# AmnonDrory/PointDSC

Hardware: AMD Instinct MI355X
Metric: correspondence-pairs/sec through NSM (N=1k/5k) at 1/2/4/8 GPUs; 3DMatch recall parity (higher is better)
Workload: dtype f32 (3xf16-split contractions); 1 GPU; synthetic random correspondences N=1000 (3dmatch-like, 30% inliers), 128 scan pairs per GPU per step, full PointDSC testing forward (12 layers x 128 ch, trained synthetic weights, classifier rescaled by synthetic.BENCH_CLS for tie-free seed ranking); num_corr=1000, global_batch=128, parallelism=dp1 (independent pairs)

## Files before the change

pointdsc_amd/csrc/attention.hip:

```cpp
#include "abi.hpp"
#include "encoder_row.hpp"

namespace pdsc {

static __global__ __launch_bounds__(256) void vexp_kernel(const float *__restrict__ v, int N, int ld, int Npad,
                                                         float *__restrict__ vexp) {
    __shared__ float part[4];
    const int t = blockIdx.x, b = blockIdx.y, tid = threadIdx.x;
    float m = 0.0f;
    for (int e = tid; e < H3_TILE * CH; e += 256) {
        const int row = t * H3_TILE + e / CH;
        if (row < N) m = fmaxf(m, fabsf(v[((size_t)b * ld + row) * CH + e % CH]));
    }
    m = wave_max(m);
    if ((tid & 63) == 0) part[tid >> 6] = m;
    __syncthreads();
    if (tid == 0) vexp[(size_t)b * (Npad / H3_TILE) + t] = (float)h3_vexp(fmaxf(fmaxf(part[0], part[1]), fmaxf(part[2], part[3])));
}

static __global__ void split_qkv_kernel(const float *__restrict__ q, const float *__restrict__ k,
                                 const float *__restrict__ v, const float *__restrict__ vexp, int B, int N,
                                 int ld, int Npad, _Float16 *__restrict__ Qs, _Float16 *__restrict__ Ks,
                                 _Float16 *__restrict__ Vs) {
    const size_t i = (size_t)blockIdx.x * blockDim.x + threadIdx.x;
// ... 13 lines not shown
    const float ev = vexp[(size_t)b * (Npad / H3_TILE) + row / H3_TILE];
    split_h(in ? ldexpf(v[src], (int)ev) : 0.0f, hi, lo);
    Vs[pb + vs_off(row, 0, c)] = hi;
    Vs[pb + vs_off(row, 1, c)] = lo;
}

hipError_t launch_attention(const EncoderPlan &plan, const void *q, const void *k, const void *v, const float *vexp,
                            const float *M, float *opart, float *ml, hipStream_t s, Ragged rg, int layer) {
    const dim3 grid(plan.workgroups());
    const _Float16 *qs = static_cast<const _Float16 *>(q), *ks = static_cast<const _Float16 *>(k),
                   *vs = static_cast<const _Float16 *>(v);
    const AttnGridH3 g = plan_grid_h3(plan, rg, layer);
    const bool packed = plan.m_layout == M_PACKED;
    switch (plan.kind) {
    case ATT_W64_SK:
        hipLaunchKernelGGL((attention_w64_sk_kernel<true>), grid, dim3(W64_NW * 64), W64_LDS, s, qs, ks, vs, vexp, M, g,
                           plan.sk_wgs, opart, ml);
        break;
    case ATT_W64:
        hipLaunchKernelGGL((attention_w64_kernel<true>), grid, dim3(W64_NW * 64), W64_LDS, s, qs, ks, vs, vexp, M, g,
                           opart, ml);
        break;
    case ATT_F32: {
        const AttnGrid gf{plan.B, plan.N, plan.Npad, plan.nqb, plan.nsplit, plan.sps, rg.nv};
        hipLaunchKernelGGL((attention_kernel_t<ATT_NW, ATT_F32_KTS, false, true>), grid, dim3(ATT_NW * 64),
                           (attention_lds_bytes<ATT_NW, ATT_F32_KTS>()), s, static_cast<const float *>(q),
                           static_cast<const float *>(k), static_cast<const float *>(v), M, gf, opart, ml);
        break;
    }
    case ATT_H3_WS:
        if (plan.vfold) return hipErrorInvalidValue;
        with_int<2, 4>(plan.ws, [&](auto ws) {
            with_bool(packed, [&](auto pk) {
                constexpr int WS = decltype(ws)::value;
                hipLaunchKernelGGL((attention_h3_ws_kernel<WS, decltype(pk)::value>), grid, dim3(WS * 64),
                                   attention_h3_ws_lds_bytes<WS>(), s, qs, ks, vs, vexp, M, g, opart, ml);
// ... 111 lines not shown
```

pointdsc_amd/csrc/attention_w64.hpp:

```cpp
#pragma once
#include "attention_h3.hpp"

namespace pdsc {

template <typename F, int... I> PDSC_DEV void static_for_(F &f, std::integer_sequence<int, I...>) {
    (f(std::integral_constant<int, I>{}), ...);
}
template <int N, typename F> PDSC_DEV void static_for(F &&f) { static_for_(f, std::make_integer_sequence<int, N>{}); }

template <typename T> PDSC_DEV void w64_pin(T &x) { asm volatile("" : "+v"(x)); }

constexpr int W64_NW = 4;
constexpr int W64_QW = 64;
constexpr int W64_QPB = W64_NW * W64_QW;
constexpr int W64_NSLOT = 4;
constexpr size_t W64_RING = (size_t)W64_NSLOT * (H3_KTB + H3_VTB);
constexpr int W64_MAXT = 1024;
constexpr size_t W64_LDS = W64_RING + W64_MAXT * sizeof(float);

constexpr int W64_AO = 0, W64_AQ = 128;
#define W64_AGPRS "a0","a1","a2","a3","a4","a5","a6","a7","a8","a9","a10","a11","a12","a13","a14","a15","a16","a17","a18","a19","a20","a21","a22","a23","a24","a25","a26","a27","a28","a29","a30","a31","a32","a33","a34","a35","a36","a37","a38","a39","a40","a41","a42","a43","a44","a45","a46","a47","a48","a49","a50","a51","a52","a53","a54","a55","a56","a57","a58","a59","a60","a61","a62","a63","a64","a65","a66","a67","a68","a69","a70","a71","a72","a73","a74","a75","a76","a77","a78","a79","a80","a81","a82","a83","a84","a85","a86","a87","a88","a89","a90","a91","a92","a93","a94","a95","a96","a97","a98","a99","a100","a101","a102","a103","a104","a105","a106","a107","a108","a109","a110","a111","a112","a113","a114","a115","a116","a117","a118","a119","a120","a121","a122","a123","a124","a125","a126","a127","a128","a129","a130","a131","a132","a133","a134","a135","a136","a137","a138","a139","a140","a141","a142","a143","a144","a145","a146","a147","a148","a149","a150","a151","a152","a153","a154","a155","a156","a157","a158","a159","a160","a161","a162","a163","a164","a165","a166","a167","a168","a169","a170","a171","a172","a173","a174","a175","a176","a177","a178","a179","a180","a181","a182","a183","a184","a185","a186","a187","a188","a189","a190","a191","a192","a193","a194","a195","a196","a197","a198","a199","a200","a201","a202","a203","a204","a205","a206","a207","a208","a209","a210","a211","a212","a213","a214","a215","a216","a217","a218","a219","a220","a221","a222","a223","a224","a225","a226","a227","a228","a229","a230","a231","a232","a233","a234","a235","a236","a237","a238","a239","a240","a241","a242","a243","a244","a245","a246","a247","a248","a249","a250","a251","a252","a253","a254","a255"
PDSC_DEV void w64_claim_agprs() { asm volatile("" ::: W64_AGPRS); }

template <int QA> PDSC_DEV void w64_kq0(f32x16 &c, const f16x8 &k) {
    asm volatile("v_mfma_f32_32x32x16_f16 %0, %1, a[%c2:%c3], 0" : "=&v"(c) : "v"(k), "i"(QA), "i"(QA + 3));
}
template <int QA> PDSC_DEV void w64_kq(f32x16 &c, const f16x8 &k) {
    asm volatile("v_mfma_f32_32x32x16_f16 %0, %1, a[%c2:%c3], %0" : "+v"(c) : "v"(k), "i"(QA), "i"(QA + 3));
}
template <int QA> PDSC_DEV void w64_kq_last(f32x16 &c, const f16x8 &k) {
    asm volatile("v_mfma_f32_32x32x16_f16 %0, %1, a[%c2:%c3], %0\n\ts_nop 11" : "+v"(c) : "v"(k), "i"(QA), "i"(QA + 3));
}
template <int U, int J> PDSC_DEV void w64_qk_step(f32x16 &S, const f16x8 (&kf)[2]) {
// ... 39 lines not shown
template <int R, int G> PDSC_DEV void w64_mload_row(__amdgpu_buffer_rsrc_t r, uint32_t voff) {
    asm volatile("buffer_load_dwordx4 v[%c0:%c1], %2, %3, 0 offen offset:%c4" ::"i"(R + 4 * G), "i"(R + 4 * G + 3),
                 "v"(voff), "s"(r), "i"(32 * G)
                 : "memory");
}
template <int R, int G> PDSC_DEV void w64_mload_col(__amdgpu_buffer_rsrc_t r, uint32_t voff) {
    asm volatile("buffer_load_dword v%c0, %4, %5, 0 offen offset:%c6\n\t"
                 "buffer_load_dword v%c1, %4, %5, 0 offen offset:%c7\n\t"
                 "buffer_load_dword v%c2, %4, %5, 0 offen offset:%c8\n\t"
                 "buffer_load_dword v%c3, %4, %5, 0 offen offset:%c9" ::"i"(R + 4 * G), "i"(R + 4 * G + 1),
                 "i"(R + 4 * G + 2), "i"(R + 4 * G + 3), "v"(voff), "s"(r), "i"(1024 * G), "i"(1024 * G + 128),
                 "i"(1024 * G + 256), "i"(1024 * G + 384)
                 : "memory");
}
template <int N> PDSC_DEV void w64_vmwait() { asm volatile("s_waitcnt vmcnt(%0)" ::"n"(N) : "memory"); }
PDSC_DEV void w64_mwait_after(bool other_keyrows) {
    if (other_keyrows)
        w64_vmwait<8 + 16>();
    else
        w64_vmwait<8 + 4>();
}
template <int R> PDSC_DEV float w64_fma_m(float sv, float mb) {
    float p;
    asm volatile("v_fma_f32 %0, v%c1, %2, -%3" : "=v"(p) : "i"(R), "v"(sv), "v"(mb));
    return p;
}
template <int R> PDSC_DEV void w64_mul_m(float &p) { asm volatile("v_mul_f32 %0, v%c1, %0" : "+v"(p) : "i"(R)); }

#ifdef W64_STAMPS
constexpr int W64_ST_PER_TILE = 6, W64_ST_TILES = 40, W64_ST_WGS = 64;
constexpr int W64_ST_PER_WAVE = W64_ST_PER_TILE * W64_ST_TILES + 8;
constexpr size_t W64_ST_LDS = (size_t)W64_NW * W64_ST_PER_WAVE * 8;
static __device__ unsigned long long g_w64_stamps[W64_ST_WGS * W64_NW * W64_ST_PER_WAVE];
#define W64_ST(i)                                                                                   \
    do {                                                                                            \
        __builtin_amdgcn_sched_barrier(0);                                                          \
// ... 9 lines not shown
    } while (0)
#endif

PDSC_DEV void w64_cvt_hi(float x0, float x1, uint32_t &hi) {
    asm volatile("v_cvt_pk_f16_f32 %0, %1, %2" : "=v"(hi) : "v"(x0), "v"(x1));
}
PDSC_DEV void w64_mix_lo(float x0, uint32_t hi, uint32_t &lo) {
    asm volatile("v_fma_mixlo_f16 %0, %1, 1.0, -%2 op_sel_hi:[0,0,1]" : "=&v"(lo) : "v"(x0), "v"(hi));
}
PDSC_DEV void w64_mix_hi(float x1, uint32_t hi, uint32_t &lo) {
    asm volatile("v_fma_mixhi_f16 %0, %1, 1.0, -%2 op_sel:[0,0,1] op_sel_hi:[0,0,1]" : "+v"(lo) : "v"(x1), "v"(hi));
}

inline AttnGridH3 attention_w64_grid(int B, int N, int slots) { return attention_h3_grid<W64_QPB / 32>(B, N, slots); }

PDSC_DEV void attention_w64_core(const _Float16 *__restrict__ Qs, const _Float16 *__restrict__ Ks,
                                 const _Float16 *__restrict__ Vs, const float *__restrict__ vexp,
                                 const float *__restrict__ M, const AttnGridH3 &g, const AttnBlock &blk, char *smem,
                                 int wave, int lane, float (&m_run)[2], float (&l_run)[2]) {
    const int b = blk.b, qb = blk.qb, split = blk.split;
    const int N = g.n(b), Npad = g.Npad;
    const int h = lane >> 5;
    const int q0 = qb * W64_QPB + wave * W64_QW;
    const int nst = (N + H3_TILE - 1) / H3_TILE;
    const int st0 = blk.st1 >= 0 ? blk.st0 : split * g.sps, st1 = blk.st1 >= 0 ? blk.st1 : min(nst, st0 + g.sps);

    const char *Kp = reinterpret_cast<const char *>(Ks + (size_t)b * Npad * 2 * CH);
    const char *Vp = reinterpret_cast<const char *>(Vs + (size_t)b * Npad * 2 * CH);
    const int mnt = mpack_ntile(g.N);
    const size_t mper = mpack_floats(g.N);
#ifdef W64_EXP_MSHARED
    const __amdgpu_buffer_rsrc_t rM = h3_rsrc(M, (uint32_t)(mper * 4u));
#else
    const __amdgpu_buffer_rsrc_t rM = h3_rsrc(M + (size_t)b * mper, (uint32_t)(mper * 4u));
#endif
    const float *vexp_b = vexp + (size_t)b * (Npad / H3_TILE);
    const __amdgpu_buffer_rsrc_t rK = h3_rsrc(Kp, (uint32_t)Npad * H3_ROWB), rV = h3_rsrc(Vp, (uint32_t)Npad * H3_ROWB);

#ifdef W64_STAMPS
    unsigned long long *st_lds = reinterpret_cast<unsigned long long *>(smem + W64_LDS) + wave * W64_ST_PER_WAVE;
    const unsigned long long st_c0 = __builtin_amdgcn_s_memtime(), st_r0 = __builtin_amdgcn_s_memrealtime();
#endif
    w64_claim_agprs();
    w64_claim_vm();
    static_for<128>([&](auto ic) { w64_zero_a<W64_AO + decltype(ic)::value>(); });
#pragma unroll
    for (int u = 0; u < 2; ++u) {
        m_run[u] = -INFINITY;
        l_run[u] = 0.0f;
    }
    if (st0 >= st1) return;
    static_for<2>([&](auto uc) {
        constexpr int u = decltype(uc)::value;
        const _Float16 *qt =
            Qs + (size_t)b * Npad * 2 * CH + (size_t)(min(q0 + 32 * u, Npad - 32) >> 5) * H3_TILE_H;
        static_for<8>([&](auto jc) {
            constexpr int j = decltype(jc)::value;
            w64_load_q<W64_AQ + 64 * u + 8 * j>(qt + h3_frag(j, 0, lane));
            w64_load_q<W64_AQ + 64 * u + 8 * j + 4>(qt + h3_frag(j, 1, lane));
        });
    });

    auto slot_of = [&](int st) { return smem + ((st - st0) & (W64_NSLOT - 1)) * (H3_KTB + H3_VTB); };
    constexpr int DMA_PW = (H3_KTB + H3_VTB) / 1024 / W64_NW;
    static_assert(H3_KTB == H3_VTB && W64_NW * DMA_PW == 2 * H3_KTB / 1024, "K / V split over the waves");
    const __amdgpu_buffer_rsrc_t rS = wave < W64_NW / 2 ? rK : rV;
    const int pbase = (wave * DMA_PW) % (H3_KTB / 1024);
    auto stage_piece = [&](int st, int i) {
        char *dst = slot_of(st) + (wave * DMA_PW + i) * 1024;
        __builtin_amdgcn_raw_ptr_buffer_load_lds(rS, (__attribute__((address_space(3))) void *)dst, 16, 16 * lane,
                                                 st * H3_KTB + (pbase + i) * 1024, 0, 0);
    };
    const int qt0 = q0 >> 5;
    const uint32_t vcol = (uint32_t)(4 * h * MPACK_T + (lane & 31)) * 4u;
    const uint32_t vrow = (uint32_t)((lane & 31) * MPACK_T + 4 * h) * 4u;
    auto keyrows = [&](int st, int u) { return st <= qt0 + u; };
    auto kr = [&](auto shc, int st, int u) {
        constexpr int SH = decltype(shc)::value;
        if constexpr (SH == 1)
            return true;
        else if constexpr (SH == 2)
            return false;
        else
            return keyrows(st, u);
    };
    using SH0 = std::integral_constant<int, 0>;
    using SH1 = std::integral_constant<int, 1>;
    using SH2 = std::integral_constant<int, 2>;
    auto load_mq = [&](auto shc, auto msc, auto uc, auto gc, int st) {
        constexpr int R = W64_VM + 32 * decltype(msc)::value + 16 * decltype(uc)::value, gg = decltype(gc)::value;
        const int qt = qt0 + decltype(uc)::value;
        if (kr(shc, st, decltype(uc)::value))
            w64_mload_col<R, gg>(rM, vcol + (uint32_t)mpack_tile(st, qt, mnt) * (MPACK_T * MPACK_T * 4u));
        else
            w64_mload_row<R, gg>(rM, vrow + (uint32_t)mpack_tile(qt, st, mnt) * (MPACK_T * MPACK_T * 4u));
    };
    const float *ev_lds = reinterpret_cast<const float *>(smem + W64_RING);
    auto load_ev = [&](int st) { return ev_lds[st]; };

#ifdef W64_EXP_NO_LDSREAD
    bool lds_once = true;
#endif
    auto kread = [&](const char *Kl, int j, f16x8(&f)[2]) {
#ifdef W64_EXP_NO_LDSREAD
        if (!lds_once) return;
#endif
        f[0] = *reinterpret_cast<const f16x8 *>(Kl + 2 * h3_frag(j, 0, lane));
        f[1] = *reinterpret_cast<const f16x8 *>(Kl + 2 * h3_frag(j, 1, lane));
    };
    auto vread = [&](const char *Vl, int i, f16x8(&f)[2]) {
#ifdef W64_EXP_NO_LDSREAD
        if (!lds_once) return;
// ... 36 lines not shown
        } else if constexpr (k == 21) {
            a.mx = halves_max(a.mx);
            w64_pin(a.mx);
        } else if constexpr (k == 22) {
            a.resc = __any(a.mx > H3_DEFER + (float)H3_PSHIFT - ev);
        }
    };
    auto rebase = [&](auto uc, SmA &a) {
        constexpr int u = decltype(uc)::value;
        if (a.resc) {
            const float m_new = fmaxf(m_run[u], a.mx + a.mb0);
            const float alpha = __builtin_amdgcn_exp2f(m_run[u] - m_new);
            const float dm = m_new - m_run[u];
            m_run[u] = m_new;
            l_run[u] *= alpha;
            static_for<64>([&](auto ic) { w64_scale_a<W64_AO + 64 * u + decltype(ic)::value>(alpha); });
            asm volatile("s_nop 1");
#pragma unroll
            for (int r = 0; r < 16; ++r) a.p[r] -= dm;
        }
    };
    auto sm1_first = [&](int u, const f32x16 &S, auto mrc, float ev, int key0, SmA &a) {
        constexpr int MR = decltype(mrc)::value;
        const float scale = ATT_QFMA ? 1.0f : H3_QSCALE;
        float mx = -INFINITY;
#pragma unroll
        for (int r = 0; r < 16; ++r) a.p[r] = S[r] * scale;
        static_for<16>([&](auto rc) { w64_mul_m<MR + decltype(rc)::value>(a.p[decltype(rc)::value]); });
        if (key0 + 32 > N) {
#pragma unroll
            for (int r = 0; r < 16; ++r)
// ... 86 lines not shown
                    w64_kq<QH>(S, f[1]);
            } else if constexpr (m == 1) {
                w64_kq<QL>(S, f[0]);
            } else {
                if constexpr (j == 7)
                    w64_kq_last<QH>(S, f[0]);
                else
                    w64_kq<QH>(S, f[0]);
            }
            slice(kc);
            __builtin_amdgcn_sched_barrier(0);
        });
    };
    auto pv_region = [&](auto uc, const char *Vl, const f16x8 (&ph)[2], const f16x8 (&pl)[2], auto nextread, auto slice) {
        constexpr int U = decltype(uc)::value;
        static_for<24>([&](auto kc) {
            constexpr int k = decltype(kc)::value, i = k / 3, m = k % 3;
            if constexpr (m == 0) {
                if constexpr (i + 2 < 8)
                    vread(Vl, i + 2, vf.f[(i + 2) % 3]);
                else
                    nextread(std::integral_constant<int, i - 6>{});
            }
            constexpr int OA = W64_AO + 64 * U + 16 * (i >> 1);
            const f16x8(&f)[2] = vf.f[i % 3];
            if constexpr (m == 0)
                w64_vp<OA>(f[0], pl[i & 1]);
            else if constexpr (m == 1)
                w64_vp<OA>(f[1], ph[i & 1]);
            else
                w64_vp<OA>(f[0], ph[i & 1]);
            slice(kc);
            __builtin_amdgcn_sched_barrier(0);
        });
    };
    auto next_k = [&](const char *Kl) { return [&, Kl](auto ic) { kread(Kl, decltype(ic)::value, kf.f[decltype(ic)::value]); }; };
    auto next_v = [&](const char *Vl) { return [&, Vl](auto ic) { vread(Vl, decltype(ic)::value, vf.f[decltype(ic)::value]); }; };
    auto none = [](auto) {};

    auto mid_barrier = [&](auto shc, int tn) {
        if (kr(shc, tn, 0))
            __builtin_amdgcn_s_waitcnt(0x4F74);
        else
            __builtin_amdgcn_s_waitcnt(0x0F78);
        __builtin_amdgcn_s_barrier();
    };

    using MSX = std::integral_constant<int, 0>;
    using MSY = std::integral_constant<int, 1>;
    auto mregs = [](auto msc, auto uc) { return std::integral_constant<int, W64_VM + 32 * decltype(msc)::value + 16 * decltype(uc)::value>{}; };
    float eX, eY;
    f32x16 S[2];
    SmA sa[2];
    SmB sb;
    f16x8 ph[2][2], pl[2][2];

    auto issue_half = [&](auto shc, auto kc, auto hc, int tn, int td, auto msn) {
        constexpr int k = decltype(kc)::value, half = decltype(hc)::value;
#ifndef W64_EXP_NO_M
        if constexpr (k % 3 == 1 && k <= 10) load_mq(shc, msn, hc, std::integral_constant<int, k / 3>{}, tn);
#endif
#ifndef W64_EXP_NO_DMA
        if constexpr (k % 3 == 1 && k >= 13) stage_piece(td, 4 * half + (k - 13) / 3);
#endif
    };
    using H0 = std::integral_constant<int, 0>;
    using H1 = std::integral_constant<int, 1>;

#pragma unroll
    for (int i = 0; i < DMA_PW; ++i) stage_piece(st0, i);
#pragma unroll
    for (int i = 0; i < DMA_PW; ++i) stage_piece(st0 + 1, i);
    static_for<2>([&](auto uc) { static_for<4>([&](auto gc) { load_mq(SH0{}, MSX{}, uc, gc, st0); }); });
    {
        float *evw = reinterpret_cast<float *>(smem + W64_RING);
        for (int i = threadIdx.x; i < Npad / H3_TILE; i += W64_NW * 64) evw[i] = vexp_b[i];
    }
    w64_vmwait<0>();
    __builtin_amdgcn_s_waitcnt(0x0070);
    __builtin_amdgcn_s_barrier();
    eX = load_ev(st0);

    {
        const int t = st0, key0 = t * H3_TILE;
        const char *L = slot_of(t);
        kread(L, 0, kf.f[0]);
        kread(L, 1, kf.f[1]);
        qk_region(std::integral_constant<int, 0>{}, L, S[0], none, none);
        static_for<24>([&](auto kc) { issue_half(SH0{}, kc, H0{}, min(t + 1, st1 - 1), t + 2, MSY{}); });
        eY = load_ev(min(t + 1, st1 - 1));
// ... 5 lines not shown
        mid_barrier(SH0{}, min(t + 1, st1 - 1));
        pv_region(std::integral_constant<int, 0>{}, L + H3_KTB, ph[0], pl[0], next_k(slot_of(t + 1)),
                  [&](auto kc) { issue_half(SH0{}, kc, H1{}, min(t + 1, st1 - 1), t + 2, MSY{}); });
        sm1_first(1, S[1], mregs(MSX{}, H1{}), eX, key0, sa[1]);
    }
    auto tile = [&](int t, auto msc, float &ec, float &ep, auto msn, float &en, auto shc) {
        const int key0 = t * H3_TILE;
        const int si = W64_ST_PER_TILE * min(t - st0, 39);
        (void)si;
        W64_ST(si);
        const char *L = slot_of(t), *Lp = slot_of(t - 1);
        qk_region(std::integral_constant<int, 0>{}, L, S[0], next_v(Lp + H3_KTB),
                  [&](auto kc) { sm2_slice(kc, 1, sa[1], ep, sb, ph[1], pl[1]); });
        W64_ST(si + 1);
        pv_region(std::integral_constant<int, 1>{}, Lp + H3_KTB, ph[1], pl[1], next_k(L), [&](auto kc) {
            if constexpr (decltype(kc)::value == 0) w64_mwait_after(kr(shc, t, 1));
            if constexpr (decltype(kc)::value == 2) en = load_ev(min(t + 1, st1 - 1));
            sm1_slice(kc, 0, S[0], mregs(msc, H0{}), ec, key0, sa[0]);
            issue_half(shc, kc, H0{}, min(t + 1, st1 - 1), t + 2, msn);
        });
        rebase(std::integral_constant<int, 0>{}, sa[0]);
        W64_ST(si + 2);
        qk_region(std::integral_constant<int, 1>{}, L, S[1], next_v(L + H3_KTB),
                  [&](auto kc) { sm2_slice(kc, 0, sa[0], ec, sb, ph[0], pl[0]); });
        W64_ST(si + 3);
        mid_barrier(shc, min(t + 1, st1 - 1));
        W64_ST(si + 4);
        pv_region(std::integral_constant<int, 0>{}, L + H3_KTB, ph[0], pl[0], next_k(slot_of(t + 1)), [&](auto kc) {
            if constexpr (decltype(kc)::value == 0) w64_mwait_after(kr(shc, min(t + 1, st1 - 1), 0));
            sm1_slice(kc, 1, S[1], mregs(msc, H1{}), ec, key0, sa[1]);
            issue_half(shc, kc, H1{}, min(t + 1, st1 - 1), t + 2, msn);
        });
        rebase(std::integral_constant<int, 1>{}, sa[1]);
        W64_ST(si + 5);
    };
#ifdef W64_EXP_NO_LDSREAD
    lds_once = false;
#endif
    int t = st0 + 1;
    for (; t + 1 < st1; t += 2) {
        auto shape = [&](int tt) { return min(tt + 1, st1 - 1) <= qt0 ? 1 : (tt >= qt0 + 2 ? 2 : 0); };
        const int s0 = shape(t), s1 = shape(t + 1);
        auto two = [&](auto shc) {
            tile(t, MSY{}, eY, eX, MSX{}, eX, shc);
// ... 29 lines not shown
        const unsigned long long st_c1 = __builtin_amdgcn_s_memtime(), st_r1 = __builtin_amdgcn_s_memrealtime();
        if (lane == 0) {
            st_lds[W64_ST_PER_WAVE - 4] = st_c0;
            st_lds[W64_ST_PER_WAVE - 3] = st_c1;
            st_lds[W64_ST_PER_WAVE - 2] = st_r0;
            st_lds[W64_ST_PER_WAVE - 1] = st_r1;
        }
        const int wg = blockIdx.x;
        if (wg < W64_ST_WGS)
            for (int i = lane; i < W64_ST_PER_WAVE; i += 64)
                g_w64_stamps[(wg * W64_NW + wave) * W64_ST_PER_WAVE + i] = st_lds[i];
    }
#endif
}

template <int U> PDSC_DEV void w64_read_o(f32x16 (&O)[4]) {
    static_for<64>([&](auto ic) {
        constexpr int i = decltype(ic)::value;
        O[i >> 4][i & 15] = w64_read_a<W64_AO + 64 * U + i>();
    });
}

PDSC_DEV void w64_store_partial(const AttnGridH3 &g, const AttnBlock &blk, float *__restrict__ opart,
                                float *__restrict__ ml, int wave, int lane, const float (&m_run)[2],
                                const float (&l_run)[2]) {
    const int Npad = g.Npad, h = lane >> 5;
    const size_t obase = (size_t)(blk.b * g.nsplit + blk.split) * Npad;
    static_for<2>([&](auto uc) {
        constexpr int u = decltype(uc)::value;
        const int q0 = blk.qb * W64_QPB + wave * W64_QW + 32 * u, qq = q0 + (lane & 31);
        f32x16 O[4];
        w64_read_o<u>(O);
        if (q0 < Npad) {
            float *Ob = opart + obase * CH + (size_t)(q0 >> 5) * (H3_TILE * CH) + 4 * lane;
#pragma unroll
            for (int t = 0; t < 4; ++t)
#pragma unroll
                for (int q = 0; q < 4; ++q)
                    *reinterpret_cast<f32x4 *>(Ob + (4 * t + q) * 256) =
                        f32x4{O[t][4 * q], O[t][4 * q + 1], O[t][4 * q + 2], O[t][4 * q + 3]};
            if (h == 0) {
                ml[(obase + qq) * 2] = (m_run[u] - (float)H3_PSHIFT) * 0.6931471805599453f;
                ml[(obase + qq) * 2 + 1] = l_run[u];
            }
        }
    });
}

template <bool XCD>
__global__ __launch_bounds__(W64_NW * 64, 1) __attribute__((amdgpu_num_vgpr(W64_VM))) void attention_w64_kernel(
    const _Float16 *__restrict__ Qs, const _Float16 *__restrict__ Ks, const _Float16 *__restrict__ Vs,
    const float *__restrict__ vexp, const float *__restrict__ M, AttnGridH3 g, float *__restrict__ opart,
    float *__restrict__ ml) {
    extern __shared__ __attribute__((aligned(16))) char w64smem[];
    const AttnBlock blk = attention_h3_block(g, XCD);
    if (blk.qb * W64_QPB >= g.n(blk.b)) return;
    const int tid = threadIdx.x, wave = __builtin_amdgcn_readfirstlane(tid >> 6), lane = tid & 63;
    float m_run[2], l_run[2];
    attention_w64_core(Qs, Ks, Vs, vexp, M, g, blk, w64smem, wave, lane, m_run, l_run);
    w64_store_partial(g, blk, opart, ml, wave, lane, m_run, l_run);
}

__host__ __device__ inline int w64_sk_owner(long x, long T, int nwg) { return (int)(((x + 1) * nwg - 1) / T); }
inline int w64_sk_nsplit(int B, int nqb, int nst, int nwg) {
    const long T = (long)B * nqb * nst;
    int ns = 1;
    for (long k = 0; k < (long)B * nqb; ++k)
        ns = std::max(ns, w64_sk_owner(k * nst + nst - 1, T, nwg) - w64_sk_owner(k * nst, T, nwg) + 1);
    return ns;
}

PDSC_DEV void w64_zero_partial(const AttnGridH3 &g, int b, int qb, int s, float *__restrict__ opart,
                               float *__restrict__ ml, int tid) {
    const int Npad = g.Npad;
    const size_t obase = (size_t)(b * g.nsplit + s) * Npad;
    const int r0 = qb * W64_QPB, r1 = min(Npad, r0 + W64_QPB);
    f32x4 *Ob = reinterpret_cast<f32x4 *>(opart + (obase + r0) * CH);
    for (int i = tid; i < (r1 - r0) * CH / 4; i += W64_NW * 64) Ob[i] = f32x4{0.0f, 0.0f, 0.0f, 0.0f};
    for (int r = r0 + tid; r < r1; r += W64_NW * 64) {
        ml[(obase + r) * 2] = -INFINITY;
        ml[(obase + r) * 2 + 1] = 0.0f;
    }
}

template <bool XCD>
__global__ __launch_bounds__(W64_NW * 64, 1) __attribute__((amdgpu_num_vgpr(W64_VM))) void attention_w64_sk_kernel(
    const _Float16 *__restrict__ Qs, const _Float16 *__restrict__ Ks, const _Float16 *__restrict__ Vs,
    const float *__restrict__ vexp, const float *__restrict__ M, AttnGridH3 g, int nwg, float *__restrict__ opart,
    float *__restrict__ ml) {
    extern __shared__ __attribute__((aligned(16))) char w64smem[];
    int w = blockIdx.x;
    if (XCD && (nwg & 7) == 0) w = (w & 7) * (nwg >> 3) + (w >> 3);
    const int nst = (g.N + H3_TILE - 1) / H3_TILE;
    const long T = (long)g.B * g.nqb * nst;
    const long hi = (long)(w + 1) * T / nwg;
    const int tid = threadIdx.x, wave = __builtin_amdgcn_readfirstlane(tid >> 6), lane = tid & 63;
    for (long x = (long)w * T / nwg; x < hi;) {
        const int k = (int)(x / nst);
        const long k0 = (long)k * nst, x1 = min(hi, k0 + nst);
        AttnBlock blk{k / g.nqb, k % g.nqb, w - w64_sk_owner(k0, T, nwg)};
        blk.st0 = (int)(x - k0);
        blk.st1 = (int)(x1 - k0);
        __builtin_amdgcn_s_waitcnt(0x0070);
        float m_run[2], l_run[2];
        attention_w64_core(Qs, Ks, Vs, vexp, M, g, blk, w64smem, wave, lane, m_run, l_run);
        w64_store_partial(g, blk, opart, ml, wave, lane, m_run, l_run);
        if (x1 == k0 + nst)
            for (int s = blk.split + 1; s < g.nsplit; ++s) w64_zero_partial(g, blk.b, blk.qb, s, opart, ml, tid);
        x = x1;
    }
}

}
```

pointdsc_amd/csrc/encoder.hip:

```cpp
#include <algorithm>
#include <cstdlib>
#include <mutex>
#include <vector>

#include "abi.hpp"
#include "encoder.hpp"
#include "pw_lds.hpp"

namespace pdsc {

static thread_local int g_diag_qkv_delay = 0;

static bool use_pw2(const Knobs &k, int B, int Npad, bool f32) {
    if (f32 || k.pw2 == 0) return false;
    return k.pw2 == 2 || (long)B * ((Npad + PW2_PTS - 1) / PW2_PTS) >= 320;
}

EncoderPlan plan_encoder(int B, int N, bool f32, bool dense_m_caller, bool allow_fused) {
    const Knobs &k = knobs();
    EncoderPlan p{};
    p.B = B;
    p.N = N;
    p.Npad = round_up(N, QB);
    p.f32 = f32;
// ... 36 lines not shown
        } else {
            p.nw = blocks <= 16 ? k.nw : ATT_NW;
            take(ATT_H3, p.nw == 1   ? attention_h3_grid<1>(B, N, k.target)
                         : p.nw == 2 ? attention_h3_grid<2>(B, N, k.target)
                                     : attention_h3_grid<ATT_NW>(B, N, k.target));
        }
        p.early = p.kind == ATT_H3 && p.sps >= 3;
    }

    p.precombine = k.precombine && !f32 && !fused && p.nsplit >= 16 && blocks <= 16;
    p.m_layout = w64 || !(f32 || dense_m_caller || k.dense_m) ? M_PACKED : M_DENSE;

    p.vfold = k.vfold && allow_fused && !f32 &&
              (fused || (p.pw2 && !p.precombine &&
                         (p.w64() || (p.kind == ATT_H3 && p.nw == ATT_NW))));
    if (fused) {
        p.kind = ATT_FUSED;
        p.nw = PW2_W;
        p.ws = 1;
        p.early = false;
        p.nqb = fg.nqb;
        p.sps = nst;
    }
    if (p.pw2) return p;

    const bool small_tiles = (long)B * (p.Npad / 64) < k.pw_small_limit;
    p.pw_tile = small_tiles ? 32 : 64;
    p.pw_mid8 = !f32 && k.pw_waves8 && (long)B * (p.Npad / 32) <= 256;
    const bool qkv3 = k.pw_qkv_split && 3L * B * (p.Npad / 32) <= 256;
    p.pw_first_qkv3 = !f32 && small_tiles && qkv3;
// ... 519 lines not shown
                split8v(v, xh[2 * t + u], xl[2 * t + u]);
            }
    }
    __syncthreads();
    w2_pcn_qkv<VFOLD>(P, pk, S, cf, d, xh, xl, featL + boff, Q + 2 * boff, K + 2 * boff, V + 2 * boff,
                      vexp + (size_t)b * (Npad / 32), row, active, wave, lane, vpad != 0);
}

template <bool VFOLD>
__global__ __launch_bounds__(PW2_W * 64, PW2_OCC) void pw2_mid_kernel(const float *__restrict__ pk, W2Sched S, PwMsg m,
                                                               PwDense4 d, const float *__restrict__ opart,
                                                               const float *__restrict__ ml, int nsplit, int N,
                                                               int Npad, const float *__restrict__ featL_in,
                                                               float *__restrict__ featL,
                                                               _Float16 *__restrict__ Q, _Float16 *__restrict__ K,
                                                               _Float16 *__restrict__ V, float *__restrict__ vexp) {
    PW2_PROLOGUE
    w2_coef_mid(cf, pk, m, d, tid, VFOLD);
    f16x8 xh[8], xl[8];
    f32x16 a2[2];
    if (active) {
        if constexpr (VFOLD)
            w2_combine_acc(opart, ml, b, nsplit, Npad, row, a2, lane);
        else
            w2_combine(opart, ml, b, nsplit, Npad, row, xh, xl, lane);
    }
    __syncthreads();
    w2_mid_chain<VFOLD>(P, pk, S, cf, m, d, xh, xl, a2, featL_in + boff, featL + boff, Q + 2 * boff, K + 2 * boff,
                        V + 2 * boff, vexp + (size_t)b * (Npad / 32), row, active, wave, lane, true);
}

template <bool PACKED, bool VFOLD>
__global__ __launch_bounds__(PW2_W * 64, PW2_OCC) void attn_pw2_kernel(
    const _Float16 *__restrict__ Qs, const _Float16 *__restrict__ Ks, const _Float16 *__restrict__ Vs,
    const float *__restrict__ vexp_in, const float *__restrict__ M, AttnGridH3 g, const float *__restrict__ pk,
    W2Sched S, PwMsg m, PwDense4 d, float *__restrict__ featL, _Float16 *__restrict__ Q, _Float16 *__restrict__ K,
    _Float16 *__restrict__ V, float *__restrict__ vexp) {
    extern __shared__ __attribute__((aligned(16))) char w2smem[];
    const AttnBlock blk = attention_h3_block(g, true);
    if (blk.qb * PW2_PTS >= g.n(blk.b)) return;
    const int b = blk.b, Npad = g.Npad, tid = threadIdx.x, wave = __builtin_amdgcn_readfirstlane(tid >> 6),
              lane = tid & 63;
    const int row = blk.qb * PW2_PTS + wave * 32 + (lane & 31);
    const bool active = blk.qb * PW2_PTS + wave * 32 < Npad;
// ... 271 lines not shown
        else                                                                                            \
            hipLaunchKernelGGL((K<64, false>), g_, dim3(256), pw_lds<64>(), s, __VA_ARGS__);            \
    } while (0)

static hipError_t launch_pw_first(const EncoderPlan &plan, const float *packed, const PackLayout &lay, const float *corr_pos,
                           float *feat, void *q, void *k, void *v, float *vexp, hipStream_t s, Ragged rg) {
    if (lay.in_dim > IN_LIMIT) return hipErrorInvalidValue;
    const int B = plan.B, N = plan.N, Npad = plan.Npad;
    _Float16 *Q = static_cast<_Float16 *>(q), *K = static_cast<_Float16 *>(k), *V = static_cast<_Float16 *>(v);
    if (plan.pw2) {
        const PwDense4 d = dense4(lay.layer[0], plan.vfold);
        const W2Sched S = sched_qkv(W2Sched{}, d, plan.vfold);
        with_bool(plan.vfold, [&](auto vf) {
            hipLaunchKernelGGL(pw2_first_kernel<decltype(vf)::value>, dim3((Npad + PW2_PTS - 1) / PW2_PTS, B),
                               dim3(PW2_W * 64), PW2_LDS, s, packed, S, lay.l0_w, lay.l0_b, d, corr_pos, lay.in_dim, N,
                               Npad, feat, Q, K, V, vexp, rg.nv, (int)!plan.fused());
        });
        return hipGetLastError();
    }
    if (plan.pw_first_qkv3) {
        hipLaunchKernelGGL((pw_first_kernel<32, false>), dim3(Npad / 32, B, 3), dim3(256), pw_lds<32>(), s, packed,
                           lay.l0_w, lay.l0_b, dense4(lay.layer[0]), corr_pos, lay.in_dim, N, Npad, feat, Q, K, V, vexp,
                           rg.nv);
        return hipGetLastError();
    }
    PW_LAUNCH(pw_first_kernel, Npad, packed, lay.l0_w, lay.l0_b, dense4(lay.layer[0]), corr_pos, lay.in_dim, N, Npad,
              feat, Q, K, V, vexp, rg.nv);
    return hipGetLastError();
}

static hipError_t launch_pw_mid(const EncoderPlan &plan, const float *packed, const PackLayout &lay, int layer,
                         const float *opart, const float *ml, int nsplit, const float *feat_in, float *feat, void *q,
                         void *k, void *v, float *vexp, hipStream_t s) {
    const int delay = g_diag_qkv_delay;
    const int B = plan.B, N = plan.N, Npad = plan.Npad;
    _Float16 *Q = static_cast<_Float16 *>(q), *K = static_cast<_Float16 *>(k), *V = static_cast<_Float16 *>(v);
    if (plan.pw2) {
        const PwMsg m = msg3(lay.layer[layer], plan.vfold);
        const PwDense4 d = dense4(lay.layer[layer + 1], plan.vfold);
        const W2Sched S = sched_qkv(sched_msg(m, plan.vfold), d, plan.vfold);
        with_bool(plan.vfold, [&](auto vf) {
            hipLaunchKernelGGL(pw2_mid_kernel<decltype(vf)::value>, dim3((Npad + PW2_PTS - 1) / PW2_PTS, B),
                               dim3(PW2_W * 64), PW2_LDS, s, packed, S, m, d, opart, ml, nsplit, N, Npad, feat_in, feat, Q,
                               K, V, vexp);
        });
        return hipGetLastError();
    }
    if (plan.pw_mid8) {
        hipLaunchKernelGGL((pw_mid_kernel<32, false, 8>), dim3(Npad / 32, B, plan.pw_mid_qkv3 ? 3 : 1), dim3(512),
                           pw_lds<32>(), s, packed,
                           msg3(lay.layer[layer]), dense4(lay.layer[layer + 1]), opart, ml, nsplit, N, Npad, feat_in,
                           feat, Q, K, V, vexp, delay, (int)plan.pw_prefetch);
        return hipGetLastError();
    }
    PW_LAUNCH(pw_mid_kernel, Npad, packed, msg3(lay.layer[layer]), dense4(lay.layer[layer + 1]), opart, ml, nsplit,
              N, Npad, feat_in, feat, Q, K, V, vexp, 0, 0);
    return hipGetLastError();
}

// ... 281 lines not shown
```

pointdsc_amd/csrc/launch_plan.hpp:

```cpp
#pragma once
#include <algorithm>
#include <cstdlib>

#include "pdsc_internal.hpp"

namespace pdsc {

constexpr int ENC_MAX_PARTS = 4;

struct Knobs {
    int target;
    int nw;
    int tiny;
    int tiny_slots;
    int ws;
    int w64;
    bool w64_sk;
    bool fuse;
    bool precombine;
    int zigzag;
    bool dense_m;
    bool vfold;
    int pw2;
    int pw_small_limit;
    bool pw_waves8;
    bool pw_qkv_split;
    bool pw_prefetch;
    int enc_halves;
    int enc_parts;
    bool enc_bal;
    bool ragged_order;
    int seed_blocks;
    bool seed_sort;
    int lm_rpt;
    int seed_select;
    bool sel_split;
    int seed_wpb;
// ... 10 lines not shown
        Knobs v;
        const int t = env_int("PDSC_ATT_TARGET", 0), nw = env_int("PDSC_ATT_NW", 2), ws = env_int("PDSC_ATT_WS", 4),
                  sl = env_int("PDSC_ATT_TINY_SLOTS", 0), wpb = env_int("PDSC_SEED_WPB", 0);
        v.target = t > 0 ? t : 512;
        v.nw = (nw == 1 || nw == 2) ? nw : 4;
        v.tiny = env_int("PDSC_ATT_TINY", 16);
        v.tiny_slots = sl > 0 ? sl : 128;
        v.ws = (ws == 1 || ws == 2) ? ws : 4;
        v.w64 = env_int("PDSC_W64", 2);
        v.w64_sk = env_int("PDSC_W64_SK", 1) != 0;
        v.fuse = env_int("PDSC_FUSE", 1) != 0;
        v.precombine = env_int("PDSC_PRECOMBINE", 1) != 0;
        v.zigzag = env_int("PDSC_ZIGZAG", 1);
        v.dense_m = env_int("PDSC_DENSE_M", 0) == 1;
        v.vfold = env_int("PDSC_VFOLD", 1) != 0;
        v.pw2 = env_int("PDSC_PW2", 1);
        v.pw_small_limit = env_int("PDSC_PW_SMALL_LIMIT", 512);
        v.pw_waves8 = env_int("PDSC_PW_WAVES", 8) != 4;
        v.pw_qkv_split = env_int("PDSC_PW_QKV_SPLIT", 1) != 0;
        v.pw_prefetch = env_int("PDSC_PW_PREFETCH", 1) != 0;
        v.enc_halves = env_int("PDSC_ENC_HALVES", 2);
        v.enc_parts = std::min(std::max(env_int("PDSC_ENC_PARTS", 2), 2), ENC_MAX_PARTS);
        v.enc_bal = env_int("PDSC_ENC_BAL", 0) == 1;
        v.ragged_order = env_int("PDSC_RAGGED_ORDER", 1) != 0;
        v.seed_blocks = env_int("PDSC_SEED_BLOCKS", 1024);
        v.seed_sort = env_int("PDSC_SEED_SORT", 0) == 1;
        v.lm_rpt = env_int("PDSC_LM_RPT", 0);
        v.seed_select = env_int("PDSC_SEED_SELECT", 2);
        v.sel_split = env_int("PDSC_SEL_SPLIT", 1) != 0;
        v.seed_wpb = (wpb == 1 || wpb == 2 || wpb == 4) ? wpb : 0;
// ... 22 lines not shown

struct EncoderPlan {
    AttnKind kind;
    int B, N, Npad;
    bool f32;
    int nw;
    int ws;
    bool early;
    int sk_wgs;
    int nqb;
    int sps;
    int nsplit;
    bool precombine;
    int m_layout;
    bool vfold;
    bool pw2;
    int pw_tile;
    bool pw_mid8;
    bool pw_first_qkv3;
    bool pw_mid_qkv3;
    bool pw_prefetch;

    bool fused() const { return kind == ATT_FUSED; }
    bool w64() const { return kind == ATT_W64 || kind == ATT_W64_SK; }

    EncoderPlan for_ragged(const Ragged &rg) const {
        EncoderPlan p = *this;
        if (kind == ATT_W64_SK && rg.nv && !rg.eq) {
            p.kind = ATT_W64;
            p.sk_wgs = 0;
        }
        return p;
    }
    EncoderPlan for_pairs(int nb) const {
        EncoderPlan p = *this;
        p.B = nb;
        return p;
    }

// ... 29 lines not shown
```

Baseline: 41.29 million correspondences/s.

## Specialise W64 attention on value width so vfold runs only the folded half-width V

Templates the W64 attention kernels on the value width CV. When vfold is active, the value tile, LDS ring slot, DMA pieces, accumulator AGPRs, PV MFMA loop and partial store shrink to CH2 columns, and the softmax slices are re-dealt over the shorter PV region. This removes loading, staging and multiplying the zero-padded upper half of V. The pointwise kernels stop writing that padding when the narrow width is selected. The main risks are the hand-tuned vmcnt waits and slice interleaving, which are re-derived from the new piece counts, and the default selects the narrow width.

New measurement: 41.23 million correspondences/s. About the same (-0.1%).

```diff
diff --git a/pointdsc_amd/csrc/attention.hip b/pointdsc_amd/csrc/attention.hip
--- a/pointdsc_amd/csrc/attention.hip
+++ b/pointdsc_amd/csrc/attention.hip
@@ -51,12 +51,17 @@
     const bool packed = plan.m_layout == M_PACKED;
     switch (plan.kind) {
     case ATT_W64_SK:
-        hipLaunchKernelGGL((attention_w64_sk_kernel<true>), grid, dim3(W64_NW * 64), W64_LDS, s, qs, ks, vs, vexp, M, g,
-                           plan.sk_wgs, opart, ml);
-        break;
     case ATT_W64:
-        hipLaunchKernelGGL((attention_w64_kernel<true>), grid, dim3(W64_NW * 64), W64_LDS, s, qs, ks, vs, vexp, M, g,
-                           opart, ml);
+        if (plan.w64_cv != CH && !(plan.w64_cv == CH2 && plan.vfold)) return hipErrorInvalidValue;
+        with_int<CH, CH2>(plan.w64_cv, [&](auto cvc) {
+            constexpr int CV = decltype(cvc)::value;
+            if (plan.kind == ATT_W64_SK)
+                hipLaunchKernelGGL((attention_w64_sk_kernel<true, CV>), grid, dim3(W64_NW * 64), w64_lds<CV>(), s, qs, ks,
+                                   vs, vexp, M, g, plan.sk_wgs, opart, ml);
+            else
+                hipLaunchKernelGGL((attention_w64_kernel<true, CV>), grid, dim3(W64_NW * 64), w64_lds<CV>(), s, qs, ks, vs,
+                                   vexp, M, g, opart, ml);
+        });
         break;
     case ATT_F32: {
         const AttnGrid gf{plan.B, plan.N, plan.Npad, plan.nqb, plan.nsplit, plan.sps, rg.nv};
diff --git a/pointdsc_amd/csrc/attention_w64.hpp b/pointdsc_amd/csrc/attention_w64.hpp
--- a/pointdsc_amd/csrc/attention_w64.hpp
+++ b/pointdsc_amd/csrc/attention_w64.hpp
@@ -14,9 +14,12 @@
 constexpr int W64_QW = 64;
 constexpr int W64_QPB = W64_NW * W64_QW;
 constexpr int W64_NSLOT = 4;
-constexpr size_t W64_RING = (size_t)W64_NSLOT * (H3_KTB + H3_VTB);
 constexpr int W64_MAXT = 1024;
-constexpr size_t W64_LDS = W64_RING + W64_MAXT * sizeof(float);
+template <int CV> constexpr int w64_vtb() { return H3_VTB * CV / CH; }
+template <int CV> constexpr int w64_slot() { return H3_KTB + w64_vtb<CV>(); }
+template <int CV> constexpr size_t w64_ring() { return (size_t)W64_NSLOT * w64_slot<CV>(); }
+template <int CV> constexpr size_t w64_lds() { return w64_ring<CV>() + W64_MAXT * sizeof(float); }
+constexpr size_t W64_LDS = w64_lds<CH>();
 
 constexpr int W64_AO = 0, W64_AQ = 128;
 #define W64_AGPRS "a0","a1","a2","a3","a4","a5","a6","a7","a8","a9","a10","a11","a12","a13","a14","a15","a16","a17","a18","a19","a20","a21","a22","a23","a24","a25","a26","a27","a28","a29","a30","a31","a32","a33","a34","a35","a36","a37","a38","a39","a40","a41","a42","a43","a44","a45","a46","a47","a48","a49","a50","a51","a52","a53","a54","a55","a56","a57","a58","a59","a60","a61","a62","a63","a64","a65","a66","a67","a68","a69","a70","a71","a72","a73","a74","a75","a76","a77","a78","a79","a80","a81","a82","a83","a84","a85","a86","a87","a88","a89","a90","a91","a92","a93","a94","a95","a96","a97","a98","a99","a100","a101","a102","a103","a104","a105","a106","a107","a108","a109","a110","a111","a112","a113","a114","a115","a116","a117","a118","a119","a120","a121","a122","a123","a124","a125","a126","a127","a128","a129","a130","a131","a132","a133","a134","a135","a136","a137","a138","a139","a140","a141","a142","a143","a144","a145","a146","a147","a148","a149","a150","a151","a152","a153","a154","a155","a156","a157","a158","a159","a160","a161","a162","a163","a164","a165","a166","a167","a168","a169","a170","a171","a172","a173","a174","a175","a176","a177","a178","a179","a180","a181","a182","a183","a184","a185","a186","a187","a188","a189","a190","a191","a192","a193","a194","a195","a196","a197","a198","a199","a200","a201","a202","a203","a204","a205","a206","a207","a208","a209","a210","a211","a212","a213","a214","a215","a216","a217","a218","a219","a220","a221","a222","a223","a224","a225","a226","a227","a228","a229","a230","a231","a232","a233","a234","a235","a236","a237","a238","a239","a240","a241","a242","a243","a244","a245","a246","a247","a248","a249","a250","a251","a252","a253","a254","a255"
@@ -86,12 +89,14 @@
                  : "memory");
 }
 template <int N> PDSC_DEV void w64_vmwait() { asm volatile("s_waitcnt vmcnt(%0)" ::"n"(N) : "memory"); }
-PDSC_DEV void w64_mwait_after(bool other_keyrows) {
+template <int PH> PDSC_DEV void w64_mwait_after(bool other_keyrows) {
     if (other_keyrows)
-        w64_vmwait<8 + 16>();
+        w64_vmwait<2 * PH + 16>();
     else
-        w64_vmwait<8 + 4>();
-}
+        w64_vmwait<2 * PH + 4>();
+}
+constexpr int w64_vmcnt_imm(int n) { return (n & 15) | ((n >> 4) << 14) | 0x0F70; }
+static_assert(w64_vmcnt_imm(20) == 0x4F74 && w64_vmcnt_imm(8) == 0x0F78, "vmcnt encoding");
 template <int R> PDSC_DEV float w64_fma_m(float sv, float mb) {
     float p;
     asm volatile("v_fma_f32 %0, v%c1, %2, -%3" : "=v"(p) : "i"(R), "v"(sv), "v"(mb));
@@ -131,6 +136,8 @@
 
 inline AttnGridH3 attention_w64_grid(int B, int N, int slots) { return attention_h3_grid<W64_QPB / 32>(B, N, slots); }
 
+constexpr int W64_DEAL12[13] = {0, 3, 6, 9, 12, 15, 17, 18, 19, 20, 21, 22, 24};
+template <int CV = CH>
 PDSC_DEV void attention_w64_core(const _Float16 *__restrict__ Qs, const _Float16 *__restrict__ Ks,
                                  const _Float16 *__restrict__ Vs, const float *__restrict__ vexp,
                                  const float *__restrict__ M, const AttnGridH3 &g, const AttnBlock &blk, char *smem,
@@ -144,6 +151,10 @@
 
     const char *Kp = reinterpret_cast<const char *>(Ks + (size_t)b * Npad * 2 * CH);
     const char *Vp = reinterpret_cast<const char *>(Vs + (size_t)b * Npad * 2 * CH);
+    static_assert(CV == CH || CV == CH2, "value width");
+    constexpr int OB = CV / 2;
+    constexpr int NF = CV / 16;
+    constexpr int SLOT = w64_slot<CV>();
     const int mnt = mpack_ntile(g.N);
     const size_t mper = mpack_floats(g.N);
 #ifdef W64_EXP_MSHARED
@@ -155,12 +166,12 @@
     const __amdgpu_buffer_rsrc_t rK = h3_rsrc(Kp, (uint32_t)Npad * H3_ROWB), rV = h3_rsrc(Vp, (uint32_t)Npad * H3_ROWB);
 
 #ifdef W64_STAMPS
-    unsigned long long *st_lds = reinterpret_cast<unsigned long long *>(smem + W64_LDS) + wave * W64_ST_PER_WAVE;
+    unsigned long long *st_lds = reinterpret_cast<unsigned long long *>(smem + w64_lds<CV>()) + wave * W64_ST_PER_WAVE;
     const unsigned long long st_c0 = __builtin_amdgcn_s_memtime(), st_r0 = __builtin_amdgcn_s_memrealtime();
 #endif
     w64_claim_agprs();
     w64_claim_vm();
-    static_for<128>([&](auto ic) { w64_zero_a<W64_AO + decltype(ic)::value>(); });
+    static_for<2 * OB>([&](auto ic) { w64_zero_a<W64_AO + decltype(ic)::value>(); });
 #pragma unroll
     for (int u = 0; u < 2; ++u) {
         m_run[u] = -INFINITY;
@@ -178,15 +189,31 @@
         });
     });
 
-    auto slot_of = [&](int st) { return smem + ((st - st0) & (W64_NSLOT - 1)) * (H3_KTB + H3_VTB); };
-    constexpr int DMA_PW = (H3_KTB + H3_VTB) / 1024 / W64_NW;
-    static_assert(H3_KTB == H3_VTB && W64_NW * DMA_PW == 2 * H3_KTB / 1024, "K / V split over the waves");
+    auto slot_of = [&](int st) { return smem + ((st - st0) & (W64_NSLOT - 1)) * SLOT; };
+    constexpr int DMA_KP = H3_KTB / 1024 / W64_NW, DMA_VP = w64_vtb<CV>() / 1024 / W64_NW;
+    constexpr int DMA_PW = DMA_KP + DMA_VP;
+    constexpr int DMA_PH = DMA_PW / 2;
+    static_assert(DMA_PW * W64_NW * 1024 == SLOT && DMA_PW % 2 == 0, "the slot's pieces over the waves and halves");
+    static_assert(H3_KTB == H3_VTB && W64_NW * 8 == 2 * H3_KTB / 1024, "K / V split over the waves");
     const __amdgpu_buffer_rsrc_t rS = wave < W64_NW / 2 ? rK : rV;
-    const int pbase = (wave * DMA_PW) % (H3_KTB / 1024);
-    auto stage_piece = [&](int st, int i) {
-        char *dst = slot_of(st) + (wave * DMA_PW + i) * 1024;
-        __builtin_amdgcn_raw_ptr_buffer_load_lds(rS, (__attribute__((address_space(3))) void *)dst, 16, 16 * lane,
-                                                 st * H3_KTB + (pbase + i) * 1024, 0, 0);
+    const int pbase = (wave * 8) % (H3_KTB / 1024);
+    auto stage_piece = [&](int st, auto ic) {
+        constexpr int I = decltype(ic)::value;
+        static_assert(I >= 0 && I < DMA_PW, "piece");
+        if constexpr (CV == CH) {
+            char *dst = slot_of(st) + (wave * DMA_PW + I) * 1024;
+            __builtin_amdgcn_raw_ptr_buffer_load_lds(rS, (__attribute__((address_space(3))) void *)dst, 16, 16 * lane,
+                                                     st * H3_KTB + (pbase + I) * 1024, 0, 0);
+        } else if constexpr (I < DMA_KP) {
+            const int piece = wave * DMA_KP + I;
+            __builtin_amdgcn_raw_ptr_buffer_load_lds(rK, (__attribute__((address_space(3))) void *)(slot_of(st) + piece * 1024),
+                                                     16, 16 * lane, st * H3_KTB + piece * 1024, 0, 0);
+        } else {
+            const int piece = wave * DMA_VP + I - DMA_KP;
+            __builtin_amdgcn_raw_ptr_buffer_load_lds(
+                rV, (__attribute__((address_space(3))) void *)(slot_of(st) + H3_KTB + piece * 1024), 16, 16 * lane,
+                st * H3_VTB + piece * 1024, 0, 0);
+        }
     };
     const int qt0 = q0 >> 5;
     const uint32_t vcol = (uint32_t)(4 * h * MPACK_T + (lane & 31)) * 4u;
@@ -212,7 +239,7 @@
         else
             w64_mload_row<R, gg>(rM, vrow + (uint32_t)mpack_tile(qt, st, mnt) * (MPACK_T * MPACK_T * 4u));
     };
-    const float *ev_lds = reinterpret_cast<const float *>(smem + W64_RING);
+    const float *ev_lds = reinterpret_cast<const float *>(smem + w64_ring<CV>());
     auto load_ev = [&](int st) { return ev_lds[st]; };
 
 #ifdef W64_EXP_NO_LDSREAD
@@ -279,7 +306,7 @@
             const float dm = m_new - m_run[u];
             m_run[u] = m_new;
             l_run[u] *= alpha;
-            static_for<64>([&](auto ic) { w64_scale_a<W64_AO + 64 * u + decltype(ic)::value>(alpha); });
+            static_for<OB>([&](auto ic) { w64_scale_a<W64_AO + OB * u + decltype(ic)::value>(alpha); });
             asm volatile("s_nop 1");
 #pragma unroll
             for (int r = 0; r < 16; ++r) a.p[r] -= dm;
@@ -396,15 +423,15 @@
     };
     auto pv_region = [&](auto uc, const char *Vl, const f16x8 (&ph)[2], const f16x8 (&pl)[2], auto nextread, auto slice) {
         constexpr int U = decltype(uc)::value;
-        static_for<24>([&](auto kc) {
+        static_for<3 * NF>([&](auto kc) {
             constexpr int k = decltype(kc)::value, i = k / 3, m = k % 3;
             if constexpr (m == 0) {
-                if constexpr (i + 2 < 8)
+                if constexpr (i + 2 < NF)
                     vread(Vl, i + 2, vf.f[(i + 2) % 3]);
                 else
-                    nextread(std::integral_constant<int, i - 6>{});
+                    nextread(std::integral_constant<int, i + 2 - NF>{});
             }
-            constexpr int OA = W64_AO + 64 * U + 16 * (i >> 1);
+            constexpr int OA = W64_AO + OB * U + 16 * (i >> 1);
             const f16x8(&f)[2] = vf.f[i % 3];
             if constexpr (m == 0)
                 w64_vp<OA>(f[0], pl[i & 1]);
@@ -412,7 +439,13 @@
                 w64_vp<OA>(f[1], ph[i & 1]);
             else
                 w64_vp<OA>(f[0], ph[i & 1]);
-            slice(kc);
+            if constexpr (NF == 8) {
+                slice(kc);
+            } else {
+                constexpr int s0 = W64_DEAL12[k];
+                static_for<W64_DEAL12[k + 1] - s0>(
+                    [&](auto jc) { slice(std::integral_constant<int, s0 + decltype(jc)::value>{}); });
+            }
             __builtin_amdgcn_sched_barrier(0);
         });
     };
@@ -422,9 +455,9 @@
 
     auto mid_barrier = [&](auto shc, int tn) {
         if (kr(shc, tn, 0))
-            __builtin_amdgcn_s_waitcnt(0x4F74);
+            __builtin_amdgcn_s_waitcnt(w64_vmcnt_imm(16 + DMA_PH));
         else
-            __builtin_amdgcn_s_waitcnt(0x0F78);
+            __builtin_amdgcn_s_waitcnt(w64_vmcnt_imm(4 + DMA_PH));
         __builtin_amdgcn_s_barrier();
     };
 
@@ -443,19 +476,18 @@
         if constexpr (k % 3 == 1 && k <= 10) load_mq(shc, msn, hc, std::integral_constant<int, k / 3>{}, tn);
 #endif
 #ifndef W64_EXP_NO_DMA
-        if constexpr (k % 3 == 1 && k >= 13) stage_piece(td, 4 * half + (k - 13) / 3);
+        if constexpr (k % 3 == 1 && k >= 13 && (k - 13) / 3 < DMA_PH)
+            stage_piece(td, std::integral_constant<int, DMA_PH * half + (k - 13) / 3>{});
 #endif
     };
     using H0 = std::integral_constant<int, 0>;
     using H1 = std::integral_constant<int, 1>;
 
-#pragma unroll
-    for (int i = 0; i < DMA_PW; ++i) stage_piece(st0, i);
-#pragma unroll
-    for (int i = 0; i < DMA_PW; ++i) stage_piece(st0 + 1, i);
+    static_for<DMA_PW>([&](auto ic) { stage_piece(st0, ic); });
+    static_for<DMA_PW>([&](auto ic) { stage_piece(st0 + 1, ic); });
     static_for<2>([&](auto uc) { static_for<4>([&](auto gc) { load_mq(SH0{}, MSX{}, uc, gc, st0); }); });
     {
-        float *evw = reinterpret_cast<float *>(smem + W64_RING);
+        float *evw = reinterpret_cast<float *>(smem + w64_ring<CV>());
         for (int i = threadIdx.x; i < Npad / H3_TILE; i += W64_NW * 64) evw[i] = vexp_b[i];
     }
     w64_vmwait<0>();
@@ -491,7 +523,7 @@
                   [&](auto kc) { sm2_slice(kc, 1, sa[1], ep, sb, ph[1], pl[1]); });
         W64_ST(si + 1);
         pv_region(std::integral_constant<int, 1>{}, Lp + H3_KTB, ph[1], pl[1], next_k(L), [&](auto kc) {
-            if constexpr (decltype(kc)::value == 0) w64_mwait_after(kr(shc, t, 1));
+            if constexpr (decltype(kc)::value == 0) w64_mwait_after<DMA_PH>(kr(shc, t, 1));
             if constexpr (decltype(kc)::value == 2) en = load_ev(min(t + 1, st1 - 1));
             sm1_slice(kc, 0, S[0], mregs(msc, H0{}), ec, key0, sa[0]);
             issue_half(shc, kc, H0{}, min(t + 1, st1 - 1), t + 2, msn);
@@ -504,7 +536,7 @@
         mid_barrier(shc, min(t + 1, st1 - 1));
         W64_ST(si + 4);
         pv_region(std::integral_constant<int, 0>{}, L + H3_KTB, ph[0], pl[0], next_k(slot_of(t + 1)), [&](auto kc) {
-            if constexpr (decltype(kc)::value == 0) w64_mwait_after(kr(shc, min(t + 1, st1 - 1), 0));
+            if constexpr (decltype(kc)::value == 0) w64_mwait_after<DMA_PH>(kr(shc, min(t + 1, st1 - 1), 0));
             sm1_slice(kc, 1, S[1], mregs(msc, H1{}), ec, key0, sa[1]);
             issue_half(shc, kc, H1{}, min(t + 1, st1 - 1), t + 2, msn);
         });
@@ -564,13 +596,14 @@
 #endif
 }
 
-template <int U> PDSC_DEV void w64_read_o(f32x16 (&O)[4]) {
-    static_for<64>([&](auto ic) {
+template <int U, int CV> PDSC_DEV void w64_read_o(f32x16 (&O)[CV / 32]) {
+    static_for<CV / 2>([&](auto ic) {
         constexpr int i = decltype(ic)::value;
-        O[i >> 4][i & 15] = w64_read_a<W64_AO + 64 * U + i>();
+        O[i >> 4][i & 15] = w64_read_a<W64_AO + CV / 2 * U + i>();
     });
 }
 
+template <int CV>
 PDSC_DEV void w64_store_partial(const AttnGridH3 &g, const AttnBlock &blk, float *__restrict__ opart,
                                 float *__restrict__ ml, int wave, int lane, const float (&m_run)[2],
                                 const float (&l_run)[2]) {
@@ -579,12 +612,12 @@
     static_for<2>([&](auto uc) {
         constexpr int u = decltype(uc)::value;
         const int q0 = blk.qb * W64_QPB + wave * W64_QW + 32 * u, qq = q0 + (lane & 31);
-        f32x16 O[4];
-        w64_read_o<u>(O);
+        f32x16 O[CV / 32];
+        w64_read_o<u, CV>(O);
         if (q0 < Npad) {
             float *Ob = opart + obase * CH + (size_t)(q0 >> 5) * (H3_TILE * CH) + 4 * lane;
 #pragma unroll
-            for (int t = 0; t < 4; ++t)
+            for (int t = 0; t < CV / 32; ++t)
 #pragma unroll
                 for (int q = 0; q < 4; ++q)
                     *reinterpret_cast<f32x4 *>(Ob + (4 * t + q) * 256) =
@@ -597,7 +630,7 @@
     });
 }
 
-template <bool XCD>
+template <bool XCD, int CV = CH>
 __global__ __launch_bounds__(W64_NW * 64, 1) __attribute__((amdgpu_num_vgpr(W64_VM))) void attention_w64_kernel(
     const _Float16 *__restrict__ Qs, const _Float16 *__restrict__ Ks, const _Float16 *__restrict__ Vs,
     const float *__restrict__ vexp, const float *__restrict__ M, AttnGridH3 g, float *__restrict__ opart,
@@ -607,8 +640,8 @@
     if (blk.qb * W64_QPB >= g.n(blk.b)) return;
     const int tid = threadIdx.x, wave = __builtin_amdgcn_readfirstlane(tid >> 6), lane = tid & 63;
     float m_run[2], l_run[2];
-    attention_w64_core(Qs, Ks, Vs, vexp, M, g, blk, w64smem, wave, lane, m_run, l_run);
-    w64_store_partial(g, blk, opart, ml, wave, lane, m_run, l_run);
+    attention_w64_core<CV>(Qs, Ks, Vs, vexp, M, g, blk, w64smem, wave, lane, m_run, l_run);
+    w64_store_partial<CV>(g, blk, opart, ml, wave, lane, m_run, l_run);
 }
 
 __host__ __device__ inline int w64_sk_owner(long x, long T, int nwg) { return (int)(((x + 1) * nwg - 1) / T); }
@@ -620,20 +653,22 @@
     return ns;
 }
 
+template <int CV>
 PDSC_DEV void w64_zero_partial(const AttnGridH3 &g, int b, int qb, int s, float *__restrict__ opart,
                                float *__restrict__ ml, int tid) {
     const int Npad = g.Npad;
     const size_t obase = (size_t)(b * g.nsplit + s) * Npad;
     const int r0 = qb * W64_QPB, r1 = min(Npad, r0 + W64_QPB);
     f32x4 *Ob = reinterpret_cast<f32x4 *>(opart + (obase + r0) * CH);
-    for (int i = tid; i < (r1 - r0) * CH / 4; i += W64_NW * 64) Ob[i] = f32x4{0.0f, 0.0f, 0.0f, 0.0f};
+    constexpr int TQ = H3_TILE * CH / 4, WQ = H3_TILE * CV / 4;
+    for (int i = tid; i < (r1 - r0) * CV / 4; i += W64_NW * 64) Ob[i / WQ * TQ + i % WQ] = f32x4{0.0f, 0.0f, 0.0f, 0.0f};
     for (int r = r0 + tid; r < r1; r += W64_NW * 64) {
         ml[(obase + r) * 2] = -INFINITY;
         ml[(obase + r) * 2 + 1] = 0.0f;
     }
 }
 
-template <bool XCD>
+template <bool XCD, int CV = CH>
 __global__ __launch_bounds__(W64_NW * 64, 1) __attribute__((amdgpu_num_vgpr(W64_VM))) void attention_w64_sk_kernel(
     const _Float16 *__restrict__ Qs, const _Float16 *__restrict__ Ks, const _Float16 *__restrict__ Vs,
     const float *__restrict__ vexp, const float *__restrict__ M, AttnGridH3 g, int nwg, float *__restrict__ opart,
@@ -653,10 +688,10 @@
         blk.st1 = (int)(x1 - k0);
         __builtin_amdgcn_s_waitcnt(0x0070);
         float m_run[2], l_run[2];
-        attention_w64_core(Qs, Ks, Vs, vexp, M, g, blk, w64smem, wave, lane, m_run, l_run);
-        w64_store_partial(g, blk, opart, ml, wave, lane, m_run, l_run);
+        attention_w64_core<CV>(Qs, Ks, Vs, vexp, M, g, blk, w64smem, wave, lane, m_run, l_run);
+        w64_store_partial<CV>(g, blk, opart, ml, wave, lane, m_run, l_run);
         if (x1 == k0 + nst)
-            for (int s = blk.split + 1; s < g.nsplit; ++s) w64_zero_partial(g, blk.b, blk.qb, s, opart, ml, tid);
+            for (int s = blk.split + 1; s < g.nsplit; ++s) w64_zero_partial<CV>(g, blk.b, blk.qb, s, opart, ml, tid);
         x = x1;
     }
 }
diff --git a/pointdsc_amd/csrc/encoder.hip b/pointdsc_amd/csrc/encoder.hip
--- a/pointdsc_amd/csrc/encoder.hip
+++ b/pointdsc_amd/csrc/encoder.hip
@@ -74,6 +74,7 @@
     p.vfold = k.vfold && allow_fused && !f32 &&
               (fused || (p.pw2 && !p.precombine &&
                          (p.w64() || (p.kind == ATT_H3 && p.nw == ATT_NW))));
+    p.w64_cv = !p.w64() ? 0 : p.vfold ? k.w64_cv : CH;
     if (fused) {
         p.kind = ATT_FUSED;
         p.nw = PW2_W;
@@ -623,7 +624,8 @@
                                                                int Npad, const float *__restrict__ featL_in,
                                                                float *__restrict__ featL,
                                                                _Float16 *__restrict__ Q, _Float16 *__restrict__ K,
-                                                               _Float16 *__restrict__ V, float *__restrict__ vexp) {
+                                                               _Float16 *__restrict__ V, float *__restrict__ vexp,
+                                                               int vpad) {
     PW2_PROLOGUE
     w2_coef_mid(cf, pk, m, d, tid, VFOLD);
     f16x8 xh[8], xl[8];
@@ -636,7 +638,7 @@
     }
     __syncthreads();
     w2_mid_chain<VFOLD>(P, pk, S, cf, m, d, xh, xl, a2, featL_in + boff, featL + boff, Q + 2 * boff, K + 2 * boff,
-                        V + 2 * boff, vexp + (size_t)b * (Npad / 32), row, active, wave, lane, true);
+                        V + 2 * boff, vexp + (size_t)b * (Npad / 32), row, active, wave, lane, vpad != 0);
 }
 
 template <bool PACKED, bool VFOLD>
@@ -938,7 +940,7 @@
         with_bool(plan.vfold, [&](auto vf) {
             hipLaunchKernelGGL(pw2_first_kernel<decltype(vf)::value>, dim3((Npad + PW2_PTS - 1) / PW2_PTS, B),
                                dim3(PW2_W * 64), PW2_LDS, s, packed, S, lay.l0_w, lay.l0_b, d, corr_pos, lay.in_dim, N,
-                               Npad, feat, Q, K, V, vexp, rg.nv, (int)!plan.fused());
+                               Npad, feat, Q, K, V, vexp, rg.nv, (int)plan.vpad());
         });
         return hipGetLastError();
     }
@@ -966,7 +968,7 @@
         with_bool(plan.vfold, [&](auto vf) {
             hipLaunchKernelGGL(pw2_mid_kernel<decltype(vf)::value>, dim3((Npad + PW2_PTS - 1) / PW2_PTS, B),
                                dim3(PW2_W * 64), PW2_LDS, s, packed, S, m, d, opart, ml, nsplit, N, Npad, feat_in, feat, Q,
-                               K, V, vexp);
+                               K, V, vexp, (int)plan.vpad());
         });
         return hipGetLastError();
     }
diff --git a/pointdsc_amd/csrc/launch_plan.hpp b/pointdsc_amd/csrc/launch_plan.hpp
--- a/pointdsc_amd/csrc/launch_plan.hpp
+++ b/pointdsc_amd/csrc/launch_plan.hpp
@@ -21,6 +21,7 @@
     int zigzag;
     bool dense_m;
     bool vfold;
+    int w64_cv;
     int pw2;
     int pw_small_limit;
     bool pw_waves8;
@@ -61,6 +62,7 @@
         v.zigzag = env_int("PDSC_ZIGZAG", 1);
         v.dense_m = env_int("PDSC_DENSE_M", 0) == 1;
         v.vfold = env_int("PDSC_VFOLD", 1) != 0;
+        v.w64_cv = env_int("PDSC_W64_CV", 64) == 128 ? 128 : 64;
         v.pw2 = env_int("PDSC_PW2", 1);
         v.pw_small_limit = env_int("PDSC_PW_SMALL_LIMIT", 512);
         v.pw_waves8 = env_int("PDSC_PW_WAVES", 8) != 4;
@@ -113,6 +115,7 @@
     bool precombine;
     int m_layout;
     bool vfold;
+    int w64_cv;
     bool pw2;
     int pw_tile;
     bool pw_mid8;
@@ -122,6 +125,7 @@
 
     bool fused() const { return kind == ATT_FUSED; }
     bool w64() const { return kind == ATT_W64 || kind == ATT_W64_SK; }
+    bool vpad() const { return vfold && w64() && w64_cv == CH; }
 
     EncoderPlan for_ragged(const Ragged &rg) const {
         EncoderPlan p = *this;
```
